# ensi321/lodestar

Hardware: AMD Instinct MI355X
Metric: verified signature sets/sec (higher is better)
Workload: dtype u32

## Files before the change

### __graft_entry__.py

```python
from __future__ import annotations

import os
import sys

ROOT = os.path.dirname(os.path.abspath(__file__))
if ROOT not in sys.path:
    sys.path.insert(0, ROOT)


def build() -> None:
    from lodestar_amd import build as b
    b.build(verbose=True)
    import oracle.bls12_381
    from oracle import build_c
    build_c.build(verbose=True)
    _build_field_selftest(b)
    from lodestar_amd.napi import build as napi_build
    if napi_build.available():
        napi_build.build(verbose=True)
    import lodestar_amd
    from lodestar_amd import native
    native.load_library()


def _build_field_selftest(b) -> None:
    import subprocess
    for name, headers in (("field_selftest", ("bls_field.h", "bls_fp_ps.h", "bls_constants.h", "bls_inv.h")),
                          ("coop_selftest", ("bls_coop.h", "bls_constants.h")),
                          ("curve_selftest", ("bls_curve.h", "bls_field.h", "bls_fp_ps.h", "bls_constants.h",
                                              "bls_inv.h")),
                          ("fr_selftest", ("bls_fr.h", "bls_constants.h"))):
        src = os.path.join(ROOT, "tests", "native", name + ".hip")
        out = os.path.join(ROOT, "tests", "native", "lib" + name + ".so")
        deps = [src] + [os.path.join(b.CSRC, h) for h in headers]
        if os.path.exists(out) and os.path.getmtime(out) >= max(os.path.getmtime(d) for d in deps):
            continue
        subprocess.check_call([b.HIPCC, f"--offload-arch={b.ARCH}", *b.FLAGS, "-shared", "-I", b.CSRC,
                               "-Wno-unused-result", "-o", out + ".tmp", src])
        os.replace(out + ".tmp", out)


def smoke() -> None:
    import hashlib

    import numpy as np

    from lodestar_amd.native import Device, pack_blobs
    from oracle import bls12_381 as O

    dev = Device(0)
    sks = [O.interop_secret_key(i) for i in range(4)]
    msgs = [hashlib.sha256(b"smoke" + bytes([i])).digest() for i in range(4)]
    pks = [O.g1_to_bytes(O.sk_to_pk(sk), compressed=False) for sk in sks]
    sigs = [O.g2_to_bytes(O.sign(sk, m)) for sk, m in zip(sks, msgs)]
    sk_be = [sk.to_bytes(32, "big") for sk in sks]
    assert dev.sign(sk_be[:2], msgs[:2]) == sigs[:2], "GPU sign != oracle"
    assert dev.sk_to_pk(sk_be[:2]) == pks[:2], "GPU sk_to_pk != oracle"
    bad_msgs = list(msgs)
    bad_msgs[3] = bytes(32)
    blob, offs = pack_blobs(sigs)
    res = dev.verify_requests(np.array([0, 3, 4], np.uint32), np.frombuffer(b"".join(pks), np.uint8), None,
                              np.frombuffer(b"".join(bad_msgs), np.uint8), blob, offs, bytes(32))
    expect = [all(O.core_verify(O.sk_to_pk(sks[i]), bad_msgs[i], O.signature_from_bytes(sigs[i]))
                  for i in range(0, 3)),
# ... 12 lines not shown
```

### lodestar_amd/build.py

```python
from __future__ import annotations

import os
import subprocess
import sys

HERE = os.path.dirname(os.path.abspath(__file__))
ROOT = os.path.dirname(HERE)
CSRC = os.path.join(HERE, "csrc")
LIB = os.path.join(HERE, "liblodestar_bls.so")
UNITS = ["k_final.hip", "k_pairing.hip", "k_aux.hip", "k_hash.hip", "k_miller.hip", "k_scalar.hip", "k_sets.hip",
         "k_smrand.hip", "k_aggsig.hip", "k_prod.hip", "k_tail.hip", "k_ssz.hip", "k_msm.hip", "k_steps.hip", "k_lp.hip",
         "k_kzg.hip", "lp_blob.hip", "bls_host.hip"]
HEADERS = ["bls_kernels.h", "bls_inv.h", "bls_field.h", "bls_fp_ps.h", "bls_curve.h", "bls_hash.h", "bls_pairing.h",
           "bls_wc12.h", "bls_wc12_tables.h", "gen_constants.py", "gen_fp_asm.py", "gen_wc12.py"]
UNIT_DEPS = {"k_lp.hip": ["bls_coop.h", "bls_lp.h", "bls_lp_progs.h"], "lp_blob.hip": ["lp_programs.bin"],
             "k_kzg.hip": ["bls_fr.h", "bls_kzg.h"],
             "bls_host.hip": ["bls_lp.h", "bls_lp_progs.h", "bls_fr.h", "bls_kzg.h"]}
LPGEN = os.path.join(HERE, "lpgen")
LP_BLOB = os.path.join(CSRC, "lp_programs.bin")
SOURCES = UNITS + HEADERS + ["bls_all.hip"] + sorted({d for v in UNIT_DEPS.values() for d in v})
OBJ_DIR = os.path.join(ROOT, "build", "obj")
HEADER = os.path.join(ROOT, "include", "lodestar_bls.h")
ARCH = os.environ.get("LB_OFFLOAD_ARCH", "gfx950")
HIPCC = os.environ.get("HIPCC", "/opt/rocm/bin/hipcc")


def _newest_source_mtime() -> float:
    paths = [os.path.join(CSRC, s) for s in SOURCES] + [HEADER, os.path.abspath(__file__)]
    return max(os.path.getmtime(p) for p in paths if os.path.exists(p))


def gen_constants() -> str:
    for header, script in (("bls_constants.h", "gen_constants.py"), ("bls_fp_ps.h", "gen_fp_asm.py"),
                           ("bls_wc12_tables.h", "gen_wc12.py")):
        out = os.path.join(CSRC, header)
        gen = os.path.join(CSRC, script)
        if not os.path.exists(out) or os.path.getmtime(out) < os.path.getmtime(gen):
            subprocess.check_call([sys.executable, gen, out])
    gen = os.path.join(CSRC, "gen_lp.py")
    srcs = [gen, os.path.join(CSRC, "gen_constants.py")] + [os.path.join(LPGEN, f) for f in os.listdir(LPGEN)
                                                            if f.endswith(".py")]
    outs = [LP_BLOB, os.path.join(CSRC, "bls_lp_progs.h")]
    if not all(os.path.exists(o) for o in outs) or min(os.path.getmtime(o) for o in outs) < max(
            os.path.getmtime(x) for x in srcs):
        subprocess.check_call([sys.executable, gen, CSRC])
    return os.path.join(CSRC, "bls_constants.h")

# ... 118 lines not shown
```

### lodestar_amd/csrc/bls_constants.h

```cpp
#pragma once
#include <stdint.h>

#define LB_P_LIMBS {0xffffaaabu, 0xb9feffffu, 0xb153ffffu, 0x1eabfffeu, 0xf6b0f624u, 0x6730d2a0u, 0xf38512bfu, 0x64774b84u, 0x434bacd7u, 0x4b1ba7b6u, 0x397fe69au, 0x1a0111eau}
#define LB_P_INV32 0xfffcfffdu
#define LB_P2_LIMBS {0xffff5556u, 0x73fdffffu, 0x62a7ffffu, 0x3d57fffdu, 0xed61ec48u, 0xce61a541u, 0xe70a257eu, 0xc8ee9709u, 0x869759aeu, 0x96374f6cu, 0x72ffcd34u, 0x340223d4u}
#define LB_P4_LIMBS {0xfffeaaacu, 0xe7fbffffu, 0xc54ffffeu, 0x7aaffffau, 0xdac3d890u, 0x9cc34a83u, 0xce144afdu, 0x91dd2e13u, 0x0d2eb35du, 0x2c6e9ed9u, 0xe5ff9a69u, 0x680447a8u}
__device__ __constant__ const uint32_t LB_ONE[12] = {0x0002fffdu, 0x76090000u, 0xc40c0002u, 0xebf4000bu, 0x53c758bau, 0x5f489857u, 0x70525745u, 0x77ce5853u, 0xa256ec6du, 0x5c071a97u, 0xfa80e493u, 0x15f65ec3u};
__device__ __constant__ const uint32_t LB_R2[12] = {0x1c341746u, 0xf4df1f34u, 0x09d104f1u, 0x0a76e6a6u, 0x4c95b6d5u, 0x8de5476cu, 0x939d83c0u, 0x67eb88a9u, 0xb519952du, 0x9a793e85u, 0x92cae3aau, 0x11988fe5u};
__device__ __constant__ const uint32_t LB_HALF[12] = {0x00015554u, 0x18040000u, 0x3ab00001u, 0x85500005u, 0x253c276fu, 0x633cb57cu, 0x31ebb502u, 0x6e22d1ecu, 0xf2d14ca2u, 0xd3916126u, 0x1a006596u, 0x17fbb857u};
#define LB_HALF_P_RAW_LIMBS {0xffffd555u, 0xdcff7fffu, 0x58a9ffffu, 0x0f55ffffu, 0x7b587b12u, 0xb3986950u, 0x79c2895fu, 0xb23ba5c2u, 0x21a5d66bu, 0x258dd3dbu, 0x1cbff34du, 0x0d0088f5u}
__device__ __constant__ const uint32_t LB_C256[12] = {0xd26ebe58u, 0xfb73eaeau, 0x3de6a351u, 0x861c2369u, 0xf951c543u, 0x76e5bc3fu, 0x6a76590cu, 0xcc0868ceu, 0x35446d0bu, 0xf0a85a3fu, 0xa49a064fu, 0x0010a8c1u};
__device__ __constant__ const uint32_t LB_B1[12] = {0x000cfff3u, 0xaa270000u, 0xfc34000au, 0x53cc0032u, 0x6b0a807fu, 0x478fe97au, 0xe6ba24d7u, 0xb1d37ebeu, 0xbf78ab2fu, 0x8ec9733bu, 0x3d83de7eu, 0x09d64551u};
__device__ __constant__ const uint32_t LB_B2[24] = {0x000cfff3u, 0xaa270000u, 0xfc34000au, 0x53cc0032u, 0x6b0a807fu, 0x478fe97au, 0xe6ba24d7u, 0xb1d37ebeu, 0xbf78ab2fu, 0x8ec9733bu, 0x3d83de7eu, 0x09d64551u, 0x000cfff3u, 0xaa270000u, 0xfc34000au, 0x53cc0032u, 0x6b0a807fu, 0x478fe97au, 0xe6ba24d7u, 0xb1d37ebeu, 0xbf78ab2fu, 0x8ec9733bu, 0x3d83de7eu, 0x09d64551u};
__device__ __constant__ const uint32_t LB_B2X3[24] = {0x0027552eu, 0x44760000u, 0x43480020u, 0xdcb8009au, 0x4a6e8b59u, 0x6f7ee9ceu, 0xc0a95bc6u, 0xb10330b7u, 0xfb1e54b7u, 0x6140b1fcu, 0x7f0bb4e1u, 0x0381be09u, 0x0027552eu, 0x44760000u, 0x43480020u, 0xdcb8009au, 0x4a6e8b59u, 0x6f7ee9ceu, 0xc0a95bc6u, 0xb10330b7u, 0xfb1e54b7u, 0x6140b1fcu, 0x7f0bb4e1u, 0x0381be09u};
#define LB_P34_WIN_STEPS 107
__device__ __constant__ const uint16_t LB_P34_WIN[107] = {1, 32, 144, 64, 99, 50, 32, 99, 82, 51, 51, 51, 65, 32, 65, 32, 48, 82, 16, 81, 67, 32, 83, 50, 50, 16, 48, 97, 32, 82, 33, 66, 16, 65, 66, 33, 49, 48, 99, 67, 32, 82, 33, 80, 83, 16, 83, 114, 64, 82, 67, 51, 49, 83, 65, 97, 32, 82, 32, 131, 50, 50, 49, 115, 50, 16, 64, 48, 131, 50, 66, 67, 51, 51, 51, 51, 33, 66, 16, 98, 32, 83, 51, 51, 51, 51, 51, 50, 33, 83, 51, 33, 67, 51, 51, 51, 51, 51, 51, 51, 51, 51, 51, 66, 66, 66, 31};
__device__ __constant__ const uint32_t LB_G1_X[12] = {0xfd530c16u, 0x5cb38790u, 0x9976fff5u, 0x7817fc67u, 0x143ba1c1u, 0x154f95c7u, 0xf3d0e747u, 0xf0ae6acdu, 0x21dbf440u, 0xedce6eccu, 0x9e0bfb75u, 0x12017741u};
__device__ __constant__ const uint32_t LB_G1_NEG_Y[12] = {0xf318883au, 0xff526c2au, 0x383b0270u, 0x92899ce4u, 0x9fa9d055u, 0x89d7738du, 0xa344c12au, 0x12caf35bu, 0x964b5317u, 0x3cff1b76u, 0xe9774430u, 0x0e44d2edu};
__device__ __constant__ const uint32_t LB_G1_Y[12] = {0x0ce72271u, 0xbaac93d5u, 0x7918fd8eu, 0x8c22631au, 0x570725ceu, 0xdd595f13u, 0x50405194u, 0x51ac5829u, 0xad0059c0u, 0x0e1c8c3fu, 0x5008a26au, 0x0bbc3efcu};
__device__ __constant__ const uint32_t LB_G1_BETA[12] = {0x798a64e8u, 0x30f1361bu, 0x7ece5a2au, 0xf3b8ddabu, 0xc61577f7u, 0x16a8ca3au, 0x74fd029bu, 0xc26a2ff8u, 0x60701c6eu, 0x3636b766u, 0x241b6160u, 0x051ba4abu};
__device__ __constant__ const uint32_t LB_PSI_CX[24] = {0x00000000u, 0x00000000u, 0x00000000u, 0x00000000u, 0x00000000u, 0x00000000u, 0x00000000u, 0x00000000u, 0x00000000u, 0x00000000u, 0x00000000u, 0x00000000u, 0x867545c3u, 0x890dc9e4u, 0x3285a5d5u, 0x2af32253u, 0x309b7e2cu, 0x50880866u, 0x7e881024u, 0xa20d1b8cu, 0xe2db9068u, 0x14e4f04fu, 0x1564853au, 0x14e56d3fu};
__device__ __constant__ const uint32_t LB_PSI_CY[24] = {0xa55c9ad1u, 0x3e2f585du, 0x86c18183u, 0x4294213du, 0x8b623732u, 0x382844c8u, 0x19103e18u, 0x92ad2afdu, 0xac7cf0b9u, 0x1d794e4fu, 0x7d825ec8u, 0x0bd592fcu, 0x5aa30fdau, 0x7bcfa7a2u, 0x2a927e7cu, 0xdc17dec1u, 0x6b4ebef1u, 0x2f088dd8u, 0xda74d4a7u, 0xd1ca2087u, 0x96cebc1du, 0x2da25966u, 0xbbfd87d2u, 0x0e2b7eedu};
__device__ __constant__ const uint32_t LB_G1_BETA2[12] = {0x8671f071u, 0xcd03c9e4u, 0x1fcda5d2u, 0x5dab2246u, 0xd3851b95u, 0x587042afu, 0x01bacb9eu, 0x8eb60ebeu, 0x83d050d2u, 0x03f97d6eu, 0x54638741u, 0x18f02065u};
__device__ __constant__ const uint32_t LB_G2_OMEGA[12] = {0x8671f071u, 0xcd03c9e4u, 0x1fcda5d2u, 0x5dab2246u, 0xd3851b95u, 0x587042afu, 0x01bacb9eu, 0x8eb60ebeu, 0x83d050d2u, 0x03f97d6eu, 0x54638741u, 0x18f02065u};
__device__ __constant__ const uint32_t LB_G2_OMEGA2[12] = {0x798a64e8u, 0x30f1361bu, 0x7ece5a2au, 0xf3b8ddabu, 0xc61577f7u, 0x16a8ca3au, 0x74fd029bu, 0xc26a2ff8u, 0x60701c6eu, 0x3636b766u, 0x241b6160u, 0x051ba4abu};
__device__ __constant__ const uint32_t LB_FROB1_1[24] = {0xb319d465u, 0x07089552u, 0xb50a8313u, 0xc6695f92u, 0xd117228fu, 0x97e83cccu, 0xb2dc29eeu, 0xa35baecau, 0x5daace4du, 0x1ce393eau, 0xb0fb66ebu, 0x08f2220fu, 0x4ce5d646u, 0xb2f66aadu, 0xfc497cecu, 0x5842a06bu, 0x2599d394u, 0xcf4895d4u, 0x40a8e8d0u, 0xc11b9cbau, 0xe5a0de89u, 0x2e3813cbu, 0x88847fafu, 0x110eefdau};
__device__ __constant__ const uint32_t LB_FROB1_2[24] = {0x00000000u, 0x00000000u, 0x00000000u, 0x00000000u, 0x00000000u, 0x00000000u, 0x00000000u, 0x00000000u, 0x00000000u, 0x00000000u, 0x00000000u, 0x00000000u, 0x8671f071u, 0xcd03c9e4u, 0x1fcda5d2u, 0x5dab2246u, 0xd3851b95u, 0x587042afu, 0x01bacb9eu, 0x8eb60ebeu, 0x83d050d2u, 0x03f97d6eu, 0x54638741u, 0x18f02065u};
__device__ __constant__ const uint32_t LB_FROB1_3[24] = {0x5aa30fdau, 0x7bcfa7a2u, 0x2a927e7cu, 0xdc17dec1u, 0x6b4ebef1u, 0x2f088dd8u, 0xda74d4a7u, 0xd1ca2087u, 0x96cebc1du, 0x2da25966u, 0xbbfd87d2u, 0x0e2b7eedu, 0x5aa30fdau, 0x7bcfa7a2u, 0x2a927e7cu, 0xdc17dec1u, 0x6b4ebef1u, 0x2f088dd8u, 0xda74d4a7u, 0xd1ca2087u, 0x96cebc1du, 0x2da25966u, 0xbbfd87d2u, 0x0e2b7eedu};
__device__ __constant__ const uint32_t LB_FROB1_4[24] = {0x867545c3u, 0x890dc9e4u, 0x3285a5d5u, 0x2af32253u, 0x309b7e2cu, 0x50880866u, 0x7e881024u, 0xa20d1b8cu, 0xe2db9068u, 0x14e4f04fu, 0x1564853au, 0x14e56d3fu, 0x00000000u, 0x00000000u, 0x00000000u, 0x00000000u, 0x00000000u, 0x00000000u, 0x00000000u, 0x00000000u, 0x00000000u, 0x00000000u, 0x00000000u, 0x00000000u};
__device__ __constant__ const uint32_t LB_FROB1_5[24] = {0x0dbce43fu, 0x82d83cf5u, 0xdf9d018fu, 0xa2813e53u, 0x3c65e181u, 0xc6f0caa5u, 0x8d50fe95u, 0x7525cf52u, 0xf4798a6bu, 0x4a85ed50u, 0x6cf8eebdu, 0x171da0fdu, 0xf242c66cu, 0x3726c30au, 0xd1b6fe70u, 0x7c2ac1aau, 0xba4b14a2u, 0xa04007fbu, 0x66341429u, 0xef517c32u, 0x4ed2226bu, 0x0095ba65u, 0xcc86f7ddu, 0x02e370ecu};
__device__ __constant__ const uint32_t LB_FROB2_1[24] = {0x798dba3au, 0xecfb361bu, 0x91865a2cu, 0xc100ddb8u, 0x232bda8eu, 0x0ec08ff1u, 0xf1ca4721u, 0xd5c13cc6u, 0xbf7b5c04u, 0x47222a47u, 0xe51c5f59u, 0x0110f184u, 0x00000000u, 0x00000000u, 0x00000000u, 0x00000000u, 0x00000000u, 0x00000000u, 0x00000000u, 0x00000000u, 0x00000000u, 0x00000000u, 0x00000000u, 0x00000000u};
__device__ __constant__ const uint32_t LB_FROB2_2[24] = {0x798a64e8u, 0x30f1361bu, 0x7ece5a2au, 0xf3b8ddabu, 0xc61577f7u, 0x16a8ca3au, 0x74fd029bu, 0xc26a2ff8u, 0x60701c6eu, 0x3636b766u, 0x241b6160u, 0x051ba4abu, 0x00000000u, 0x00000000u, 0x00000000u, 0x00000000u, 0x00000000u, 0x00000000u, 0x00000000u, 0x00000000u, 0x00000000u, 0x00000000u, 0x00000000u, 0x00000000u};
__device__ __constant__ const uint32_t LB_FROB2_3[24] = {0xfffcaaaeu, 0x43f5ffffu, 0xed47fffdu, 0x32b7fff2u, 0xa2e99d69u, 0x07e83a49u, 0x8332bb7au, 0xeca8f331u, 0xa0f4c069u, 0xef148d1eu, 0x3eff0206u, 0x040ab326u, 0x00000000u, 0x00000000u, 0x00000000u, 0x00000000u, 0x00000000u, 0x00000000u, 0x00000000u, 0x00000000u, 0x00000000u, 0x00000000u, 0x00000000u, 0x00000000u};
__device__ __constant__ const uint32_t LB_FROB2_4[24] = {0x8671f071u, 0xcd03c9e4u, 0x1fcda5d2u, 0x5dab2246u, 0xd3851b95u, 0x587042afu, 0x01bacb9eu, 0x8eb60ebeu, 0x83d050d2u, 0x03f97d6eu, 0x54638741u, 0x18f02065u, 0x00000000u, 0x00000000u, 0x00000000u, 0x00000000u, 0x00000000u, 0x00000000u, 0x00000000u, 0x00000000u, 0x00000000u, 0x00000000u, 0x00000000u, 0x00000000u};
__device__ __constant__ const uint32_t LB_FROB2_5[24] = {0x867545c3u, 0x890dc9e4u, 0x3285a5d5u, 0x2af32253u, 0x309b7e2cu, 0x50880866u, 0x7e881024u, 0xa20d1b8cu, 0xe2db9068u, 0x14e4f04fu, 0x1564853au, 0x14e56d3fu, 0x00000000u, 0x00000000u, 0x00000000u, 0x00000000u, 0x00000000u, 0x00000000u, 0x00000000u, 0x00000000u, 0x00000000u, 0x00000000u, 0x00000000u, 0x00000000u};
__device__ __constant__ const uint32_t LB_FROB3_1[24] = {0xa55c9ad1u, 0x3e2f585du, 0x86c18183u, 0x4294213du, 0x8b623732u, 0x382844c8u, 0x19103e18u, 0x92ad2afdu, 0xac7cf0b9u, 0x1d794e4fu, 0x7d825ec8u, 0x0bd592fcu, 0x5aa30fdau, 0x7bcfa7a2u, 0x2a927e7cu, 0xdc17dec1u, 0x6b4ebef1u, 0x2f088dd8u, 0xda74d4a7u, 0xd1ca2087u, 0x96cebc1du, 0x2da25966u, 0xbbfd87d2u, 0x0e2b7eedu};
__device__ __constant__ const uint32_t LB_FROB3_2[24] = {0x00000000u, 0x00000000u, 0x00000000u, 0x00000000u, 0x00000000u, 0x00000000u, 0x00000000u, 0x00000000u, 0x00000000u, 0x00000000u, 0x00000000u, 0x00000000u, 0x0002fffdu, 0x76090000u, 0xc40c0002u, 0xebf4000bu, 0x53c758bau, 0x5f489857u, 0x70525745u, 0x77ce5853u, 0xa256ec6du, 0x5c071a97u, 0xfa80e493u, 0x15f65ec3u};
__device__ __constant__ const uint32_t LB_FROB3_3[24] = {0xa55c9ad1u, 0x3e2f585du, 0x86c18183u, 0x4294213du, 0x8b623732u, 0x382844c8u, 0x19103e18u, 0x92ad2afdu, 0xac7cf0b9u, 0x1d794e4fu, 0x7d825ec8u, 0x0bd592fcu, 0xa55c9ad1u, 0x3e2f585du, 0x86c18183u, 0x4294213du, 0x8b623732u, 0x382844c8u, 0x19103e18u, 0x92ad2afdu, 0xac7cf0b9u, 0x1d794e4fu, 0x7d825ec8u, 0x0bd592fcu};
__device__ __constant__ const uint32_t LB_FROB3_4[24] = {0xfffcaaaeu, 0x43f5ffffu, 0xed47fffdu, 0x32b7fff2u, 0xa2e99d69u, 0x07e83a49u, 0x8332bb7au, 0xeca8f331u, 0xa0f4c069u, 0xef148d1eu, 0x3eff0206u, 0x040ab326u, 0x00000000u, 0x00000000u, 0x00000000u, 0x00000000u, 0x00000000u, 0x00000000u, 0x00000000u, 0x00000000u, 0x00000000u, 0x00000000u, 0x00000000u, 0x00000000u};
__device__ __constant__ const uint32_t LB_FROB3_5[24] = {0x5aa30fdau, 0x7bcfa7a2u, 0x2a927e7cu, 0xdc17dec1u, 0x6b4ebef1u, 0x2f088dd8u, 0xda74d4a7u, 0xd1ca2087u, 0x96cebc1du, 0x2da25966u, 0xbbfd87d2u, 0x0e2b7eedu, 0xa55c9ad1u, 0x3e2f585du, 0x86c18183u, 0x4294213du, 0x8b623732u, 0x382844c8u, 0x19103e18u, 0x92ad2afdu, 0xac7cf0b9u, 0x1d794e4fu, 0x7d825ec8u, 0x0bd592fcu};
__device__ __constant__ const uint32_t LB_SSWU_A[24] = {0x00000000u, 0x00000000u, 0x00000000u, 0x00000000u, 0x00000000u, 0x00000000u, 0x00000000u, 0x00000000u, 0x00000000u, 0x00000000u, 0x00000000u, 0x00000000u, 0x03135242u, 0xe53a0000u, 0xdef80285u, 0x01080c0fu, 0xe340f6bdu, 0xe7889edbu, 0x26310601u, 0x0b513751u, 0x17c744abu, 0x02d69857u, 0x79ea5467u, 0x1220b4e9u};
__device__ __constant__ const uint32_t LB_SSWU_B[24] = {0x0cf89db2u, 0x22ea0000u, 0x71380aa4u, 0x6ec832dfu, 0x3db5a66eu, 0x6e1b9440u, 0xa79473bau, 0x75bf3c53u, 0x412c0a34u, 0x3dd3a569u, 0x74dc4fd1u, 0x125cdb5eu, 0x0cf89db2u, 0x22ea0000u, 0x71380aa4u, 0x6ec832dfu, 0x3db5a66eu, 0x6e1b9440u, 0xa79473bau, 0x75bf3c53u, 0x412c0a34u, 0x3dd3a569u, 0x74dc4fd1u, 0x125cdb5eu};
__device__ __constant__ const uint32_t LB_SSWU_Z[24] = {0xfff9555cu, 0x87ebffffu, 0xda8ffffau, 0x656fffe5u, 0x45d33ad2u, 0x0fd07493u, 0x066576f4u, 0xd951e663u, 0x41e980d3u, 0xde291a3du, 0x7dfe040du, 0x0815664cu, 0xfffcaaaeu, 0x43f5ffffu, 0xed47fffdu, 0x32b7fff2u, 0xa2e99d69u, 0x07e83a49u, 0x8332bb7au, 0xeca8f331u, 0xa0f4c069u, 0xef148d1eu, 0x3eff0206u, 0x040ab326u};
__device__ __constant__ const uint32_t LB_SSWU_MINUS_B_OVER_A[24] = {0x55474fb3u, 0x903c5555u, 0xce451105u, 0x5f98cc95u, 0xefe0fadeu, 0x9f8e582eu, 0xaebbd062u, 0xc68946b6u, 0x0ee6de53u, 0x467a4ad1u, 0x83e23a05u, 0x0e7146f4u, 0xaab85af8u, 0x29c2aaaau, 0xe30eeefau, 0xbf133368u, 0x06cffb45u, 0xc7a27a72u, 0x44c9425cu, 0x9dee04ceu, 0x3464ce83u, 0x04a15ce5u, 0xb59dac95u, 0x0b8fcaf5u};
__device__ __constant__ const uint32_t LB_SSWU_B_OVER_ZA[24] = {0x44414324u, 0xf2d84444u, 0x93a69d00u, 0x2585c283u, 0x5d972c42u, 0x5dd35cd0u, 0x4ea89b53u, 0xfd963b74u, 0x91c1fa91u, 0x07f5d9fdu, 0x3ce062c4u, 0x127db28au, 0x333b3695u, 0x55743333u, 0x590828fcu, 0xeb72b871u, 0xcb4d5da5u, 0x1c186171u, 0xee956644u, 0x34a33031u, 0x149d16d0u, 0xc971692au, 0xf5de8b82u, 0x168a1e1fu};
__device__ __constant__ const uint32_t LB_SSWU_NZ3_SQRT[12] = {0x7c72b3a1u, 0xd5ebd442u, 0x2ddcd3e5u, 0x1cd49652u, 0x81eec7dfu, 0xbef2fbb7u, 0x7bd484bfu, 0xa7e8879du, 0x147c4f33u, 0x8ae5e5b2u, 0xba7795dau, 0x12c7e800u};
__device__ __constant__ const uint32_t LB_ISO_XNUM0[24] = {0x1ce05e62u, 0x47f671c7u, 0x1206393eu, 0x06dd5707u, 0xf3fd71a2u, 0x7c80cd2au, 0x9e6cd062u, 0x048103eau, 0xc8d037f6u, 0xc54516acu, 0x0920ea41u, 0x13808f55u, 0x1ce05e62u, 0x47f671c7u, 0x1206393eu, 0x06dd5707u, 0xf3fd71a2u, 0x7c80cd2au, 0x9e6cd062u, 0x048103eau, 0xc8d037f6u, 0xc54516acu, 0x0920ea41u, 0x13808f55u};
__device__ __constant__ const uint32_t LB_ISO_XNUM1[24] = {0x00000000u, 0x00000000u, 0x00000000u, 0x00000000u, 0x00000000u, 0x00000000u, 0x00000000u, 0x00000000u, 0x00000000u, 0x00000000u, 0x00000000u, 0x00000000u, 0x554c71d0u, 0x5fe55555u, 0x236aaaa3u, 0x873fffddu, 0xb26ef918u, 0x6a6b4619u, 0x08874945u, 0x21c28884u, 0x028cabc5u, 0x2836cda7u, 0xa7fd5abdu, 0x0ac73310u};
__device__ __constant__ const uint32_t LB_ISO_XNUM2[24] = {0x555971c3u, 0x0a0c5555u, 0x1f9eaaaeu, 0xdb0c0010u, 0x1d797997u, 0xb1fb2f94u, 0xef416e1cu, 0xd3960742u, 0xc20556f4u, 0xb70040e2u, 0xe581393bu, 0x149d7861u, 0xaaa638e8u, 0xaff2aaaau, 0x91b55551u, 0x439fffeeu, 0xd9377c8cu, 0xb535a30cu, 0x0443a4a2u, 0x90e14442u, 0x814655e2u, 0x941b66d3u, 0x53fead5eu, 0x05639988u};
// ... 23 lines not shown
```

### lodestar_amd/csrc/bls_field.h

```cpp
#pragma once
#include <hip/hip_runtime.h>
#include <stdint.h>

#include "bls_constants.h"
#include "bls_inv.h"

#define LB_DEV __device__ __forceinline__
#define LB_NOINL __device__ __noinline__
#ifndef LB_TOWER_NOINLINE
#define LB_TOWER LB_DEV
#else
#define LB_TOWER LB_NOINL
#endif

namespace lb {

struct fp {
  uint32_t l[12];
};
struct fp2 {
  fp c0, c1;
};
struct fp6 {
  fp2 c0, c1, c2;
// ... 30 lines not shown
#pragma unroll
  for (int j = 0; j < 12; j++) r.l[j] = c ? a.l[j] : r.l[j];
}

LB_DEV void fp_csub_p(fp& r, const uint32_t* t) {
  uint32_t s[12];
  uint32_t br = 0;
#pragma unroll
  for (int j = 0; j < 12; j++) s[j] = __builtin_subc(t[j], P_[j], br, &br);
#pragma unroll
  for (int j = 0; j < 12; j++) r.l[j] = br ? t[j] : s[j];
}

#include "bls_fp_ps.h"

LB_DEV void fp_add(fp& r, const fp& a, const fp& b) { fp_add_ps(r, a, b); }
LB_DEV void fp_sub(fp& r, const fp& a, const fp& b) { fp_sub_ps(r, a, b); }
LB_DEV void fp_dbl(fp& r, const fp& a) { fp_add_ps(r, a, a); }
LB_DEV void fp_neg(fp& r, const fp& a) {
  fp z;
  fp_zero(z);
  fp_sub_ps(r, z, a);
}

#ifdef LB_COUNT_OPS
__device__ unsigned long long g_lb_fpmul_count;
#define LB_COUNT_MUL() atomicAdd(&g_lb_fpmul_count, 2ull)
#define LB_COUNT_HALF() atomicAdd(&g_lb_fpmul_count, 1ull)
#define LB_COUNT_SQR() atomicAdd(&g_lb_fpmul_count, 1ull << 32)
#else
#define LB_COUNT_MUL() ((void)0)
#define LB_COUNT_HALF() ((void)0)
#define LB_COUNT_SQR() ((void)0)
#endif

struct fp_ret {
  uint32_t v0, v1, v2, v3, v4, v5, v6, v7, v8, v9, v10, v11;
};
#define LB_FP_PARAMS(x)                                                                                   \
  uint32_t x##0, uint32_t x##1, uint32_t x##2, uint32_t x##3, uint32_t x##4, uint32_t x##5, uint32_t x##6, \
      uint32_t x##7, uint32_t x##8, uint32_t x##9, uint32_t x##10, uint32_t x##11
#define LB_FP_PACK(x) {{x##0, x##1, x##2, x##3, x##4, x##5, x##6, x##7, x##8, x##9, x##10, x##11}}
#define LB_FP_ARGS(f) \
  f.l[0], f.l[1], f.l[2], f.l[3], f.l[4], f.l[5], f.l[6], f.l[7], f.l[8], f.l[9], f.l[10], f.l[11]

LB_NOINL fp_ret fp_mul_r(LB_FP_PARAMS(a), LB_FP_PARAMS(b)) {
  LB_COUNT_MUL();
  const fp A = LB_FP_PACK(a), B = LB_FP_PACK(b);
  fp r;
  fp_mul_ps_body(r, A, B);
  return fp_ret{r.l[0], r.l[1], r.l[2], r.l[3], r.l[4], r.l[5], r.l[6], r.l[7], r.l[8], r.l[9], r.l[10], r.l[11]};
}
LB_NOINL fp_ret fp_sqr_r(LB_FP_PARAMS(a)) {
  LB_COUNT_SQR();
  const fp A = LB_FP_PACK(a);
  fp r;
  fp_sqr_ps_body(r, A);
  return fp_ret{r.l[0], r.l[1], r.l[2], r.l[3], r.l[4], r.l[5], r.l[6], r.l[7], r.l[8], r.l[9], r.l[10], r.l[11]};
}
LB_DEV void fp_unret(fp& r, const fp_ret& v) {
  r.l[0] = v.v0;
  r.l[1] = v.v1;
  r.l[2] = v.v2;
  r.l[3] = v.v3;
  r.l[4] = v.v4;
  r.l[5] = v.v5;
// ... 33 lines not shown
  fp r;
  fp_redc_ps_body(r, W);
  return fp_ret{r.l[0], r.l[1], r.l[2], r.l[3], r.l[4], r.l[5], r.l[6], r.l[7], r.l[8], r.l[9], r.l[10], r.l[11]};
}
LB_DEV void fpw_unret(uint32_t* w, const fpw_ret& v) {
#pragma unroll
  for (int j = 0; j < 24; j++) w[j] = v[j];
}
LB_DEV void fp_mulw(uint32_t* w, const fp& a, const fp& b) { fpw_unret(w, fp_mulw_r(LB_FP_ARGS(a), LB_FP_ARGS(b))); }
LB_DEV void fp_redc(fp& r, const uint32_t* w) { fp_unret(r, fp_redc_r(LB_W_ARGS(w))); }
LB_DEV void fp_sqr(fp& r, const fp& a) { fp_unret(r, fp_sqr_r(LB_FP_ARGS(a))); }

LB_DEV void fp_mul_const(fp& r, const fp& a, const uint32_t* c) {
  fp k;
  fp_set(k, c);
  fp_mul(r, a, k);
}

LB_DEV void fp_to_mont(fp& r, const fp& a) { fp_mul_const(r, a, LB_R2); }
LB_DEV void fp_from_mont(fp& r, const fp& a) {
  fp one_raw;
  fp_zero(one_raw);
  one_raw.l[0] = 1;
  fp_mul(r, a, one_raw);
}

LB_DEV void fp_mul3(fp& r, const fp& a) {
  fp t;
  fp_add(t, a, a);
  fp_add(r, t, a);
}

LB_NOINL fp_ret fp_pow_p34_r(LB_FP_PARAMS(x)) {
  fp t1 = LB_FP_PACK(x), a2, t3, t5, t7;
  fp_sqr(a2, t1);
  fp_mul(t3, t1, a2);
  fp_mul(t5, t3, a2);
  fp_mul(t7, t5, a2);
  fp acc;
  switch (LB_P34_WIN[0] & 15) {
    case 0: acc = t1; break;
    case 1: acc = t3; break;
    case 2: acc = t5; break;
    default: acc = t7; break;
  }
#pragma unroll 1
  for (int k = 1; k < LB_P34_WIN_STEPS; k++) {
    const uint32_t st = LB_P34_WIN[k];
#pragma unroll 1
    for (uint32_t q = st >> 4; q > 0; q--) fp_sqr(acc, acc);
    switch (st & 15) {
      case 0: fp_mul(acc, acc, t1); break;
      case 1: fp_mul(acc, acc, t3); break;
      case 2: fp_mul(acc, acc, t5); break;
      case 3: fp_mul(acc, acc, t7); break;
      default: break;
    }
  }
  return fp_ret{acc.l[0], acc.l[1], acc.l[2], acc.l[3], acc.l[4], acc.l[5],
                acc.l[6], acc.l[7], acc.l[8], acc.l[9], acc.l[10], acc.l[11]};
}
LB_DEV void fp_pow_p34(fp& r, const fp& a) { fp_unret(r, fp_pow_p34_r(LB_FP_ARGS(a))); }

LB_NOINL fp_ret fp_inv_r(LB_FP_PARAMS(a)) {
#ifdef LB_COUNT_OPS
  atomicAdd(&g_lb_fpmul_count, 20ull);
#endif
  const uint32_t y[12] = {a0, a1, a2, a3, a4, a5, a6, a7, a8, a9, a10, a11};
  uint32_t w[12];
  lb_inv::inv_raw(w, y);
  fp t, c;
#pragma unroll
  for (int j = 0; j < 12; j++) {
    t.l[j] = w[j];
    c.l[j] = lb_inv::R3[j];
  }
  fp r;
  fp_mul(r, t, c);
  return fp_ret{r.l[0], r.l[1], r.l[2], r.l[3], r.l[4], r.l[5], r.l[6], r.l[7], r.l[8], r.l[9], r.l[10], r.l[11]};
}
LB_DEV void fp_inv(fp& r, const fp& a) { fp_unret(r, fp_inv_r(LB_FP_ARGS(a))); }

LB_DEV bool fp_is_square(const fp& a) {
  fp t, one;
  fp_pow_p34(t, a);
  fp_sqr(t, t);
  fp_mul(t, t, a);
  fp_one(one);
  return fp_is_zero(a) || fp_eq(t, one);
}

LB_DEV bool fp_sqrt(fp& r, const fp& a) {
  fp t, s2;
// ... 498 lines not shown
```

### lodestar_amd/csrc/gen_constants.py

```python
import os
import sys

P = 0x1A0111EA397FE69A4B1BA7B6434BACD764774B84F38512BF6730D2A0F6B0F6241EABFFFEB153FFFFB9FEFFFFFFFFAAAB
R_ORDER = 0x73EDA753299D7D483339D80809A1D80553BDA402FFFE5BFEFFFFFFFF00000001
X_ABS = 0xD201000000010000
MONT_R = 1 << 384
NL = 12


def limbs(v, n=NL):
    return [(v >> (32 * i)) & 0xFFFFFFFF for i in range(n)]


def mont(v):
    return (v % P) * MONT_R % P


VALUES = {}


def c_fp(name, v, raw=False):
    VALUES[name] = v if raw else v % P
    vals = limbs(v % P if not raw else v)
    if not raw:
# ... 89 lines not shown
    if not VALUES:
        main(None)
    return dict(VALUES)


def main(out_path):
    lines = [
        "// GENERATED by gen_constants.py -- do not edit.",
        "#pragma once",
        "#include <stdint.h>",
        "",
    ]
    lines.append("#define LB_P_LIMBS {" + ", ".join("0x%08xu" % x for x in limbs(P)) + "}")
    n0 = (-pow(P, -1, 1 << 32)) % (1 << 32)
    lines.append("#define LB_P_INV32 0x%08xu  // -p^-1 mod 2^32" % n0)
    lines.append("#define LB_P2_LIMBS {" + ", ".join("0x%08xu" % x for x in limbs(2 * P)) + "}")
    lines.append("#define LB_P4_LIMBS {" + ", ".join("0x%08xu" % x for x in limbs(4 * P)) + "}")
    lines.append(c_fp("LB_ONE", 1))
    lines.append(c_fp("LB_R2", MONT_R * MONT_R % P, raw=True).replace("LB_R2", "LB_R2"))
    lines[-1] = "__device__ __constant__ const uint32_t LB_R2[12] = {%s};" % ", ".join(
        "0x%08xu" % x for x in limbs(MONT_R * MONT_R % P))
    lines.append(c_fp("LB_HALF", (P + 1) // 2))
    lines.append("#define LB_HALF_P_RAW_LIMBS {" + ", ".join("0x%08xu" % x for x in limbs((P - 1) // 2)) + "}")
    lines.append("__device__ __constant__ const uint32_t LB_C256[12] = {%s};" % ", ".join(
        "0x%08xu" % x for x in limbs(pow(2, 256 + 768, P))))
    lines.append(c_fp("LB_B1", 4))
    lines.append(c_fp2("LB_B2", (4, 4)))
    lines.append(c_fp2("LB_B2X3", (12, 12)))
    check_p34_window_program()
    prog = p34_window_program(3)
    lines.append("#define LB_P34_WIN_STEPS %d" % len(prog))
    lines.append("__device__ __constant__ const uint16_t LB_P34_WIN[%d] = {%s};" % (
        len(prog), ", ".join(str(x) for x in prog)))
    g1x = 0x17F1D3A73197D7942695638C4FA9AC0FC3688C4F9774B905A14E3A3F171BAC586C55E83FF97A1AEFFB3AF00ADB22C6BB
    g1y = 0x08B3F481E3AAA0F1A09E30ED741D8AE4FCF5E095D5D00AF600DB18CB2C04B3EDD03CC744A2888AE40CAA232946C5E7E1
    lines.append(c_fp("LB_G1_X", g1x))
    lines.append(c_fp("LB_G1_NEG_Y", (-g1y) % P))
    lines.append(c_fp("LB_G1_Y", g1y))
    cands = []
    g = 2
    while len(cands) < 1:
        c = pow(g, (P - 1) // 3, P)
        if c != 1:
            cands = [c, c * c % P]
        g += 1

    def g1add(p1, p2):
        if p1 is None:
            return p2
        if p2 is None:
            return p1
        if p1[0] == p2[0]:
            if (p1[1] + p2[1]) % P == 0:
                return None
            lam = 3 * p1[0] * p1[0] * pow(2 * p1[1], P - 2, P) % P
        else:
            lam = (p2[1] - p1[1]) * pow(p2[0] - p1[0], P - 2, P) % P
        x3 = (lam * lam - p1[0] - p2[0]) % P
        return (x3, (lam * (p1[0] - x3) - p1[1]) % P)

    def g1mul(pt, k):
        acc = None
        for b in bin(k)[2:]:
            acc = g1add(acc, acc)
            if b == "1":
                acc = g1add(acc, pt)
# ... 90 lines not shown
```

Before: 3.705 million.

## Compute p-3/4 exponentiation in 30-bit limb Montgomery domain

Replaces the (p-3)/4 power used for square roots with a version that converts the input into 13 limbs of 30 bits and runs Montgomery multiply/square with lazy 64-bit column accumulation, so carries are deferred instead of propagated per step. A precomputed exit constant folds the domain conversion (Montgomery R factor correction) into one final multiply, and the result is converted back to 32-bit limbs. This targets the cost of the long square-and-multiply chain in hash-to-curve and decompression. In exchange it adds a second field representation with extra conversion code, more column multiplies (13x13 versus 12x12), and possibly more register pressure.

```diff
diff --git a/__graft_entry__.py b/__graft_entry__.py
--- a/__graft_entry__.py
+++ b/__graft_entry__.py
@@ -25,11 +25,14 @@
 
 def _build_field_selftest(b) -> None:
     import subprocess
-    for name, headers in (("field_selftest", ("bls_field.h", "bls_fp_ps.h", "bls_constants.h", "bls_inv.h")),
+    for name, headers in (("field_selftest", ("bls_field.h", "bls_fp_ps.h", "bls_fp_pow.h", "bls_constants.h",
+                                              "bls_inv.h")),
                           ("coop_selftest", ("bls_coop.h", "bls_constants.h")),
-                          ("curve_selftest", ("bls_curve.h", "bls_field.h", "bls_fp_ps.h", "bls_constants.h",
-                                              "bls_inv.h")),
-                          ("fr_selftest", ("bls_fr.h", "bls_constants.h"))):
+                          ("curve_selftest", ("bls_curve.h", "bls_field.h", "bls_fp_ps.h", "bls_fp_pow.h",
+                                              "bls_constants.h", "bls_inv.h")),
+                          ("fr_selftest", ("bls_fr.h", "bls_constants.h")),
+                          ("pow_selftest", ("bls_fp_pow.h", "bls_field.h", "bls_fp_ps.h", "bls_constants.h",
+                                            "bls_inv.h"))):
         src = os.path.join(ROOT, "tests", "native", name + ".hip")
         out = os.path.join(ROOT, "tests", "native", "lib" + name + ".so")
         deps = [src] + [os.path.join(b.CSRC, h) for h in headers]
diff --git a/lodestar_amd/build.py b/lodestar_amd/build.py
--- a/lodestar_amd/build.py
+++ b/lodestar_amd/build.py
@@ -11,8 +11,8 @@
 UNITS = ["k_final.hip", "k_pairing.hip", "k_aux.hip", "k_hash.hip", "k_miller.hip", "k_scalar.hip", "k_sets.hip",
          "k_smrand.hip", "k_aggsig.hip", "k_prod.hip", "k_tail.hip", "k_ssz.hip", "k_msm.hip", "k_steps.hip", "k_lp.hip",
          "k_kzg.hip", "lp_blob.hip", "bls_host.hip"]
-HEADERS = ["bls_kernels.h", "bls_inv.h", "bls_field.h", "bls_fp_ps.h", "bls_curve.h", "bls_hash.h", "bls_pairing.h",
-           "bls_wc12.h", "bls_wc12_tables.h", "gen_constants.py", "gen_fp_asm.py", "gen_wc12.py"]
+HEADERS = ["bls_kernels.h", "bls_inv.h", "bls_field.h", "bls_fp_ps.h", "bls_fp_pow.h", "bls_curve.h", "bls_hash.h",
+           "bls_pairing.h", "bls_wc12.h", "bls_wc12_tables.h", "gen_constants.py", "gen_fp_asm.py", "gen_wc12.py"]
 UNIT_DEPS = {"k_lp.hip": ["bls_coop.h", "bls_lp.h", "bls_lp_progs.h"], "lp_blob.hip": ["lp_programs.bin"],
              "k_kzg.hip": ["bls_fr.h", "bls_kzg.h"],
              "bls_host.hip": ["bls_lp.h", "bls_lp_progs.h", "bls_fr.h", "bls_kzg.h"]}
diff --git a/lodestar_amd/csrc/bls_constants.h b/lodestar_amd/csrc/bls_constants.h
--- a/lodestar_amd/csrc/bls_constants.h
+++ b/lodestar_amd/csrc/bls_constants.h
@@ -15,6 +15,7 @@
 __device__ __constant__ const uint32_t LB_B2X3[24] = {0x0027552eu, 0x44760000u, 0x43480020u, 0xdcb8009au, 0x4a6e8b59u, 0x6f7ee9ceu, 0xc0a95bc6u, 0xb10330b7u, 0xfb1e54b7u, 0x6140b1fcu, 0x7f0bb4e1u, 0x0381be09u, 0x0027552eu, 0x44760000u, 0x43480020u, 0xdcb8009au, 0x4a6e8b59u, 0x6f7ee9ceu, 0xc0a95bc6u, 0xb10330b7u, 0xfb1e54b7u, 0x6140b1fcu, 0x7f0bb4e1u, 0x0381be09u};
 #define LB_P34_WIN_STEPS 107
 __device__ __constant__ const uint16_t LB_P34_WIN[107] = {1, 32, 144, 64, 99, 50, 32, 99, 82, 51, 51, 51, 65, 32, 65, 32, 48, 82, 16, 81, 67, 32, 83, 50, 50, 16, 48, 97, 32, 82, 33, 66, 16, 65, 66, 33, 49, 48, 99, 67, 32, 82, 33, 80, 83, 16, 83, 114, 64, 82, 67, 51, 49, 83, 65, 97, 32, 82, 32, 131, 50, 50, 49, 115, 50, 16, 64, 48, 131, 50, 66, 67, 51, 51, 51, 51, 33, 66, 16, 98, 32, 83, 51, 51, 51, 51, 51, 50, 33, 83, 51, 33, 67, 51, 51, 51, 51, 51, 51, 51, 51, 51, 51, 66, 66, 66, 31};
+#define LB_POW_EXIT30 {0x3fff5556u, 0x0ff7ffffu, 0x2a7ffff7u, 0x15ffff58u, 0x21ec483du, 0x069507b5u, 0x2257ece6u, 0x25c279c2u, 0x19aec8eeu, 0x3db21a5du, 0x13496374u, 0x351cbff3u, 0x00140223u}
 __device__ __constant__ const uint32_t LB_G1_X[12] = {0xfd530c16u, 0x5cb38790u, 0x9976fff5u, 0x7817fc67u, 0x143ba1c1u, 0x154f95c7u, 0xf3d0e747u, 0xf0ae6acdu, 0x21dbf440u, 0xedce6eccu, 0x9e0bfb75u, 0x12017741u};
 __device__ __constant__ const uint32_t LB_G1_NEG_Y[12] = {0xf318883au, 0xff526c2au, 0x383b0270u, 0x92899ce4u, 0x9fa9d055u, 0x89d7738du, 0xa344c12au, 0x12caf35bu, 0x964b5317u, 0x3cff1b76u, 0xe9774430u, 0x0e44d2edu};
 __device__ __constant__ const uint32_t LB_G1_Y[12] = {0x0ce72271u, 0xbaac93d5u, 0x7918fd8eu, 0x8c22631au, 0x570725ceu, 0xdd595f13u, 0x50405194u, 0x51ac5829u, 0xad0059c0u, 0x0e1c8c3fu, 0x5008a26au, 0x0bbc3efcu};
diff --git a/lodestar_amd/csrc/bls_field.h b/lodestar_amd/csrc/bls_field.h
--- a/lodestar_amd/csrc/bls_field.h
+++ b/lodestar_amd/csrc/bls_field.h
@@ -86,6 +86,15 @@
 #define LB_COUNT_MUL() ((void)0)
 #define LB_COUNT_HALF() ((void)0)
 #define LB_COUNT_SQR() ((void)0)
+#endif
+
+#ifndef LB_POW_COLS
+#define LB_POW_COLS 1
+#endif
+#if LB_POW_COLS
+}
+#include "bls_fp_pow.h"
+namespace lb {
 #endif
 
 struct fp_ret {
@@ -185,6 +194,12 @@
 }
 
 LB_NOINL fp_ret fp_pow_p34_r(LB_FP_PARAMS(x)) {
+#if LB_POW_COLS
+  const uint32_t a[12] = {x0, x1, x2, x3, x4, x5, x6, x7, x8, x9, x10, x11};
+  uint32_t r[12];
+  pw::pow_p34(r, a);
+  return fp_ret{r[0], r[1], r[2], r[3], r[4], r[5], r[6], r[7], r[8], r[9], r[10], r[11]};
+#else
   fp t1 = LB_FP_PACK(x), a2, t3, t5, t7;
   fp_sqr(a2, t1);
   fp_mul(t3, t1, a2);
@@ -212,6 +227,7 @@
   }
   return fp_ret{acc.l[0], acc.l[1], acc.l[2], acc.l[3], acc.l[4], acc.l[5],
                 acc.l[6], acc.l[7], acc.l[8], acc.l[9], acc.l[10], acc.l[11]};
+#endif
 }
 LB_DEV void fp_pow_p34(fp& r, const fp& a) { fp_unret(r, fp_pow_p34_r(LB_FP_ARGS(a))); }
 
diff --git a/lodestar_amd/csrc/bls_fp_pow.h b/lodestar_amd/csrc/bls_fp_pow.h
--- /dev/null
+++ b/lodestar_amd/csrc/bls_fp_pow.h
@@ -0,0 +1,157 @@
+#pragma once
+#include <stdint.h>
+
+#ifndef LB_HD
+#define LB_HD __device__ __forceinline__
+#endif
+#ifndef LB_COUNT_MUL
+#define LB_COUNT_MUL() ((void)0)
+#define LB_COUNT_SQR() ((void)0)
+#endif
+
+namespace lb {
+namespace pw {
+
+constexpr uint32_t M30 = (1u << 30) - 1;
+
+struct d13 {
+  uint32_t d[13];
+};
+constexpr d13 p_digits() {
+  constexpr uint32_t P32[12] = LB_P_LIMBS;
+  d13 r{};
+  for (int i = 0; i < 13; i++) {
+    const int o = 30 * i, w = o / 32, s = o % 32;
+    const uint64_t v = (uint64_t)(w < 12 ? P32[w] : 0u) | ((uint64_t)(w + 1 < 12 ? P32[w + 1] : 0u) << 32);
+    r.d[i] = (uint32_t)(v >> s) & M30;
+  }
+  return r;
+}
+constexpr uint32_t p_inv30() {
+  constexpr d13 P = p_digits();
+  uint32_t inv = 1;
+  for (int k = 0; k < 6; k++) inv *= 2u - P.d[0] * inv;
+  return (0u - inv) & M30;
+}
+constexpr d13 PD = p_digits();
+constexpr uint32_t PINV30 = p_inv30();
+static_assert(((PD.d[0] * PINV30) & M30) == M30, "-p^-1 mod 2^30");
+constexpr d13 EXIT = {LB_POW_EXIT30};
+
+LB_HD void enter(d13& r, const uint32_t* a) {
+#pragma unroll
+  for (int i = 0; i < 13; i++) {
+    const int o = 30 * i, w = o / 32, s = o % 32;
+    const uint32_t lo = a[w] >> s;
+    const uint32_t hi = (s > 2 && w + 1 < 12) ? a[w + 1] << (32 - s) : 0u;
+    r.d[i] = (lo | hi) & M30;
+  }
+}
+LB_HD void leave(uint32_t* r, const d13& a) {
+  constexpr uint32_t P32[12] = LB_P_LIMBS;
+  uint32_t t[12], s[12];
+#pragma unroll
+  for (int j = 0; j < 12; j++) {
+    const int o = 32 * j, k = o / 30, sh = o % 30;
+    uint32_t v = a.d[k] >> sh;
+    v |= a.d[k + 1] << (30 - sh);
+    t[j] = v;
+  }
+  uint32_t br = 0;
+#pragma unroll
+  for (int j = 0; j < 12; j++) {
+    const uint64_t d = (uint64_t)t[j] - P32[j] - br;
+    s[j] = (uint32_t)d;
+    br = (uint32_t)(d >> 63);
+  }
+#pragma unroll
+  for (int j = 0; j < 12; j++) r[j] = br ? t[j] : s[j];
+}
+
+template <bool SQR>
+LB_HD void mont(d13& r, const d13& a, const d13& b) {
+  uint32_t a2[13], m[13];
+  if (SQR) {
+#pragma unroll
+    for (int i = 0; i < 13; i++) a2[i] = a.d[i] << 1;
+  }
+  uint64_t cp = 0, cr = 0;
+#pragma unroll
+  for (int k = 0; k < 26; k++) {
+    const int i0 = k < 13 ? 0 : k - 12, i1 = k < 13 ? k : 12;
+    uint64_t ap = cp, ar = cr;
+    if (SQR) {
+#pragma unroll
+      for (int i = i0; 2 * i < k; i++) ap += (uint64_t)a2[i] * a.d[k - i];
+      if (k % 2 == 0 && k <= 24) ap += (uint64_t)a.d[k / 2] * a.d[k / 2];
+    } else {
+#pragma unroll
+      for (int i = i0; i <= i1; i++) ap += (uint64_t)a.d[i] * b.d[k - i];
+    }
+#pragma unroll
+    for (int i = i0; i <= i1 && i < k; i++) ar += (uint64_t)m[i] * PD.d[k - i];
+    if (k < 13) {
+      m[k] = (((uint32_t)ap + (uint32_t)ar) * PINV30) & M30;
+      ar += (uint64_t)m[k] * PD.d[0];
+    }
+    ar += (uint32_t)ap & M30;
+    if (k >= 13) r.d[k - 13] = (uint32_t)ar & M30;
+    cp = ap >> 30;
+    cr = ar >> 30;
+  }
+}
+LB_HD void mul(d13& r, const d13& a, const d13& b) { mont<false>(r, a, b); }
+LB_HD void sqr(d13& r, const d13& a) { mont<true>(r, a, a); }
+
+LB_HD void pow_p34(uint32_t* r, const uint32_t* a) {
+  enum { T1 = 0, T3 = 1, T5 = 2, T7 = 3, AUX = 4, NONE = 15 };
+  d13 t1, t3, t5, t7, aux, acc;
+  enter(t1, a);
+  acc = aux = t3 = t5 = t7 = t1;
+#pragma unroll 1
+  for (int k = -4; k <= LB_P34_WIN_STEPS; k++) {
+    uint32_t st;
+    if (k == -4) st = (1u << 4) | NONE;
+    else if (k == -3) st = T1;
+    else if (k < 0) st = AUX;
+    else if (k == 0) st = NONE;
+    else if (k < LB_P34_WIN_STEPS) st = LB_P34_WIN[k];
+    else st = AUX;
+#pragma unroll 1
+    for (uint32_t q = st >> 4; q > 0; q--) {
+      LB_COUNT_SQR();
+      sqr(acc, acc);
+    }
+    d13 m = t1;
+    bool product = true;
+    switch (st & 15) {
+      case T1: break;
+      case T3: m = t3; break;
+      case T5: m = t5; break;
+      case T7: m = t7; break;
+      case AUX: m = aux; break;
+      default: product = false; break;
+    }
+    if (product) {
+      if (k < LB_P34_WIN_STEPS) LB_COUNT_MUL();
+      mul(acc, acc, m);
+    }
+    if (k == -4) aux = acc;
+    else if (k == -3) t3 = acc;
+    else if (k == -2) t5 = acc;
+    else if (k == -1) t7 = acc;
+    else if (k == 0) {
+      aux = EXIT;
+      switch (LB_P34_WIN[0] & 15) {
+        case 0: acc = t1; break;
+        case 1: acc = t3; break;
+        case 2: acc = t5; break;
+        default: acc = t7; break;
+      }
+    }
+  }
+  leave(r, acc);
+}
+
+}
+}
diff --git a/lodestar_amd/csrc/gen_constants.py b/lodestar_amd/csrc/gen_constants.py
--- a/lodestar_amd/csrc/gen_constants.py
+++ b/lodestar_amd/csrc/gen_constants.py
@@ -145,6 +145,9 @@
     lines.append("#define LB_P34_WIN_STEPS %d" % len(prog))
     lines.append("__device__ __constant__ const uint16_t LB_P34_WIN[%d] = {%s};" % (
         len(prog), ", ".join(str(x) for x in prog)))
+    pow_exit = pow(2, 384 + 6 * ((P - 3) // 4), P)
+    lines.append("#define LB_POW_EXIT30 {" + ", ".join(
+        "0x%08xu" % ((pow_exit >> (30 * i)) & ((1 << 30) - 1)) for i in range(13)) + "}")
     g1x = 0x17F1D3A73197D7942695638C4FA9AC0FC3688C4F9774B905A14E3A3F171BAC586C55E83FF97A1AEFFB3AF00ADB22C6BB
     g1y = 0x08B3F481E3AAA0F1A09E30ED741D8AE4FCF5E095D5D00AF600DB18CB2C04B3EDD03CC744A2888AE40CAA232946C5E7E1
     lines.append(c_fp("LB_G1_X", g1x))
```

Result: faster. 3.925 million (median of 6 runs) (+5.9%).
